# TRI-ML/sdflabel

Hardware: AMD Instinct MI355X
Metric: rendered rays/sec (fwd+bwd) (higher is better)
Workload: dtype f32; 1 GPU; BASELINE configs[1]: one 256x256 crop(s) per GPU, DeepSDF 8x512 on a 40^3 grid, fwd+bwd to yaw/trans/latent, decoder re-evaluated every step; crops_per_gpu=1, rays_per_crop=65536, grid_points=64000, surfels=2751, front_facing=763, parallelism=crop-parallel x1

## Files before the change

### sdflabel_amd/csrc/kcj_slots.h

```cpp
#pragma once
#include <stdint.h>
#if defined(__HIPCC__) || defined(__CUDACC__)
#define SDFR_KCJ_HD __host__ __device__ __forceinline__
#else
#define SDFR_KCJ_HD inline
#endif

constexpr int SDFR_KCJ_PT = 16;
constexpr int SDFR_KCJ_KT = 16;
constexpr int SDFR_KCJ_RING = 4;

SDFR_KCJ_HD int sdfr_kcj_popc(uint32_t x) { return __builtin_popcount(x); }
SDFR_KCJ_HD int sdfr_kcj_count(uint32_t w0, uint32_t w1, uint32_t w2, uint32_t w3) {
    return sdfr_kcj_popc(w0) + sdfr_kcj_popc(w1) + sdfr_kcj_popc(w2) + sdfr_kcj_popc(w3);
}
SDFR_KCJ_HD int sdfr_kcj_rank(uint32_t w0, uint32_t w1, uint32_t w2, uint32_t w3, int q, int g) {
    const uint32_t below = (uint32_t)((1ull << q) - 1ull);
    int r = sdfr_kcj_popc(w0 & below) + sdfr_kcj_popc(w1 & below) + sdfr_kcj_popc(w2 & below) + sdfr_kcj_popc(w3 & below);
    if (g > 0) r += (int)((w0 >> q) & 1u);
    if (g > 1) r += (int)((w1 >> q) & 1u);
    if (g > 2) r += (int)((w2 >> q) & 1u);
    return r;
}
SDFR_KCJ_HD int sdfr_kcj_feature(int q, int g) { return (q >> 2) * 16 + 4 * g + (q & 3); }
SDFR_KCJ_HD int sdfr_kcj_vec(int pos) { return (pos >> 4) * 4 + (pos & 3); }
SDFR_KCJ_HD int sdfr_kcj_comp(int pos) { return (pos & 15) >> 2; }
SDFR_KCJ_HD int sdfr_kcj_elem(int pos, int point) { return (sdfr_kcj_vec(pos) * SDFR_KCJ_PT + point) * 4 + sdfr_kcj_comp(pos); }
SDFR_KCJ_HD int sdfr_kcj_kidx(int pos) { return sdfr_kcj_vec(pos) * 4 + sdfr_kcj_comp(pos); }
SDFR_KCJ_HD int sdfr_kcj_padded(int tot) {
    const int trip = SDFR_KCJ_KT * SDFR_KCJ_RING;
    const int p = (tot + trip - 1) / trip * trip;
    return p < trip ? trip : p;
}
SDFR_KCJ_HD int sdfr_kcj_pad_pos(int tot, int e) { return tot + e / SDFR_KCJ_PT; }
SDFR_KCJ_HD int sdfr_kcj_pad_point(int e) { return e % SDFR_KCJ_PT; }

SDFR_KCJ_HD int sdfr_kcj_col(int j) { return (j & ~127) | ((j & 15) << 3) | ((j >> 4) & 7); }

SDFR_KCJ_HD int sdfr_kcj_ring_clamp(int tile, int nkt) { return tile < nkt ? tile : nkt - 1; }
SDFR_KCJ_HD int sdfr_kcj_ring_gather_tile(int t, int nkt) { return sdfr_kcj_ring_clamp(t + SDFR_KCJ_RING - 1, nkt); }
SDFR_KCJ_HD int sdfr_kcj_ring_klist_tile(int t, int nkt) { return sdfr_kcj_ring_clamp(t + SDFR_KCJ_RING, nkt); }
SDFR_KCJ_HD int sdfr_kcj_ring_operand_tile(int t, int nkt) { return sdfr_kcj_ring_clamp(t + 1, nkt); }
```

### sdflabel_amd/csrc/mlp_kernel.h

```cpp
#pragma once
#include "sdfr_common.h"
#include "kc_slots.h"
#include "kcj_slots.h"
#include "tile_balance.h"
#include <math.h>
#include <type_traits>

typedef float f32x16 __attribute__((ext_vector_type(16)));
typedef float f32x4 __attribute__((ext_vector_type(4)));
typedef _Float16 h16;
typedef h16 h16x8 __attribute__((ext_vector_type(8)));
typedef h16 h16x4 __attribute__((ext_vector_type(4)));

struct MlpLayer {
    int in_dim, out_dim;
    int inj_n, inj_off;
    int kp_f, kp_b, kp_h;
    int off_f, off_b, off_h;
    int kp_bh, off_bh;
    int kp_s, off_s;
    int ln;
};

struct MlpParams {
// ... 106 lines not shown
    static constexpr int KV = 4, NSTEP = 4;
    static __device__ __forceinline__ acc_t step(const vec_t& a, const vec_t& b, acc_t c, int ks) {
        return __builtin_amdgcn_mfma_f32_16x16x4f32(f4c(a, ks), f4c(b, ks), c, 0, 0, 0);
    }
};
template <> struct Mma<h16, 32> {
    typedef f32x16 acc_t; typedef h16x8 vec_t;
    static constexpr int KV = 8, NSTEP = 1;
    static __device__ __forceinline__ acc_t step(const vec_t& a, const vec_t& b, acc_t c, int) {
#ifdef SDFR_ABL_NOMFMA
        c[0] += (float)a[0] * (float)b[0];
        return c;
#else
        return __builtin_amdgcn_mfma_f32_32x32x16_f16(a, b, c, 0, 0, 0);
#endif
    }
};
template <> struct Mma<h16, 16> {
    typedef f32x4 acc_t; typedef h16x8 vec_t;
    static constexpr int KV = 8, NSTEP = 1;
    static __device__ __forceinline__ acc_t step(const vec_t& a, const vec_t& b, acc_t c, int) {
        return __builtin_amdgcn_mfma_f32_16x16x32_f16(a, b, c, 0, 0, 0);
    }
};
__device__ __forceinline__ void store4(float* dst, const float* v) { *reinterpret_cast<float4*>(dst) = make_float4(v[0], v[1], v[2], v[3]); }
__device__ __forceinline__ void store4(h16* dst, const float* v) {
    h16x4 t; t[0] = (h16)v[0]; t[1] = (h16)v[1]; t[2] = (h16)v[2]; t[3] = (h16)v[3];
    *reinterpret_cast<h16x4*>(dst) = t;
}

__device__ __forceinline__ int64_t sdfr_mask_dword(int64_t r, int l, int n_layers, int HP32, int j) {
    return (((r >> 7) * n_layers + l) * 128 + (r & 127)) * HP32 + (j >> 5);
}
__host__ __device__ __forceinline__ int sdfr_wk_row(int r) { return (r & ~63) | ((r & 31) << 1) | ((r >> 5) & 1); }
__device__ __forceinline__ int sdfr_mask_shift(int j) { return ((j >> 2) & 1) * 16 + ((j & 31) >> 3) * 4 + (j & 3); }

#ifndef SDFR_MLP_WPE
#define SDFR_MLP_WPE 1
#endif
template <typename ET, int MS, int FT, int NP, int NW, int MODE, bool LN, int XF> constexpr bool sdfr_mlp_kc() {
    return sizeof(ET) == 4 && MS == 32 && FT == 2 && NP == 2 && NW == 8 && (MODE == 0 || MODE == 1) && !LN && (XF & ~4) == 0;
}
template <typename ET, int MS, int FT, int NP, int NW, int MODE, bool LN, int XF> constexpr bool sdfr_mlp_kcj() {
    return sizeof(ET) == 4 && MS == 16 && NP == 1 && NW == 4 && FT == 8 && MODE == 3 && !LN && XF == 0;
}
template <typename ET, int MS, int FT, int NP, int NW, int PF, int MODE, int PFB_ = 0, bool LN = false, int XF = 0>
__global__ __launch_bounds__(64 * NW, SDFR_MLP_WPE) void sdfr_mlp_kernel(const MlpParams P) {
    typedef Mma<ET, MS> M;
    typedef typename M::acc_t acc_t;
    typedef typename M::vec_t vec_t;
    constexpr bool HALF = sizeof(ET) == 2;
    constexpr bool JAC = MODE == 2 || MODE == 3;
    constexpr bool TAIL = MODE == 4;
    constexpr bool SAVE = MODE == 1;
    constexpr bool LMASK = MODE == 2;
    constexpr bool GMASK = MODE == 3;
    constexpr bool GATHER = (XF & 1) != 0;
    constexpr bool PERSIST = (XF & 2) != 0;
    constexpr bool ORDER = (XF & 4) != 0;
    static_assert(!ORDER || (XF == 4 && (MODE == 0 || MODE == 1) && sizeof(ET) == 4 && MS == 32 && FT == 2), "ORDER: the exact-f32 grid forward alone");
    static_assert(XF == 0 || (MODE == 0 || MODE == 1) || (MODE == 3 && XF == 2), "GATHER is a forward feature; PERSIST: forward modes and the mask-fed Jacobian");
    constexpr bool JPOOL = JAC && PERSIST;
    static_assert(!SAVE || MS == 32, "mask layout assumes 32x32 forward tiles");
    static_assert(!SAVE || (FT * NP) % 2 == 0, "mask words: FT*NP*16 bits per thread and layer must fill whole words");
    static_assert(!HALF || !JAC || MODE == 3, "with half operands only the mask-fed Jacobian exists (MODE 3)");
    static_assert(!LN || (!HALF && MODE != 1 && MODE != 3 && MODE != 4), "LayerNorm decoders: float32 forward (MODE 0) and recomputing Jacobian (MODE 2)");
    static_assert(!TAIL || (NP * MS <= 64 && (NP * MS) % 16 == 0), "tail march: the tile's rows (t_rt rays x K samples) live in wave 0");
    constexpr int KV = M::KV;
    constexpr int NLG = 64 / MS;
    constexpr int RG = MS / (4 * NLG);
    constexpr int KT = KV * NLG;
    constexpr int NT = 64 * NW;
    constexpr int PT = MS * NP;
    constexpr int HP = MS * FT * NW;
    constexpr int KG = HP / KV;
    constexpr int FT32 = HP / (32 * NW);
    constexpr int MW = (FT * NP * RG * 4 + 31) / 32;
    constexpr int MASK_WORDS = LMASK ? (SDFR_MAX_LAYERS * MW * NT) : 1;
    constexpr int LN_F4 = LN ? (NW * PT + SDFR_MAX_LAYERS * PT + 3) / 4 : 0;
    constexpr int KGX = KG + ((HALF && !JAC) ? 4 : 0);
    constexpr bool DBUF = HALF && !JAC && !LN && !SAVE && (2 * KGX * PT * 16 <= 144 * 1024);
    constexpr bool KC = sdfr_mlp_kc<ET, MS, FT, NP, NW, MODE, LN, XF>();
    constexpr int KZ4 = KC ? SDFR_KCD_ROW_BYTES / 16 : 0;
    constexpr int ACT4 = (DBUF ? 2 : 1) * KGX * PT + KZ4;
    constexpr bool MLDS = GMASK && HALF && MS == 16 && HP == 512;
    static_assert(!MLDS || (FT == 4 && NW == 8), "MLDS: a wave owns 64 features = two mask dwords of a row");
    constexpr int MLDS_WORDS = MLDS ? NW * SDFR_MAX_LAYERS * PT * 2 : 0;
    constexpr int O_RED = ACT4, O_ROWS = O_RED + NT / 4, O_GY = O_ROWS + 32, O_SLOTS = O_GY + (PT + 3) / 4, O_MASKS = O_SLOTS + (PT + 3) / 4;
    constexpr int O_LN = O_MASKS + (MASK_WORDS + 3) / 4, O_MLDS = O_LN + LN_F4, LDS4 = O_MLDS + (MLDS_WORDS + 3) / 4;
    __shared__ float4 lds4[LDS4];
    vec_t* act = reinterpret_cast<vec_t*>(lds4);
    ET* act_e = reinterpret_cast<ET*>(lds4);
    vec_t* actw = DBUF ? act + KGX * PT : act;
    ET* actw_e = reinterpret_cast<ET*>(actw);
    float* red = reinterpret_cast<float*>(lds4 + O_RED);
    int* rows = reinterpret_cast<int*>(lds4 + O_ROWS);
    float* gy = reinterpret_cast<float*>(lds4 + O_GY);
    int* slots = reinterpret_cast<int*>(lds4 + O_SLOTS);
    uint32_t* masks = reinterpret_cast<uint32_t*>(lds4 + O_MASKS);
    float* lnred = reinterpret_cast<float*>(lds4 + O_LN);
    float* lnrstd = lnred + NW * PT;
    uint32_t* mlds = reinterpret_cast<uint32_t*>(lds4 + O_MLDS);
    __shared__ float jinj[MLDS ? PT * 8 : 1];
    __shared__ int jpfx[JPOOL ? 66 : 1];
    __shared__ int4 kc_list4[KC ? HP / 4 : 1];
    __shared__ int4 kc_cnt4[KC ? NW / 4 : 1];
    int* kc_cnt = reinterpret_cast<int*>(kc_cnt4);
    static_assert(!KC || (KGX * PT * 16 == SDFR_KCD_ZERO_ROW * SDFR_KCD_ROW_BYTES && HP == SDFR_KCD_WK_ROW_FLOATS),
                  "kc_slots.h: the dense image is 512 rows of 256 bytes, its zero row right behind it");
    static_assert(!KC || (KT == 8 && KV == 4 && NW == 8), "kc_slots.h: k tiles of 8, vectors of 4, 8 waves");
    constexpr bool KCJ = sdfr_mlp_kcj<ET, MS, FT, NP, NW, MODE, LN, XF>();
    __shared__ int4 kcj_list4[KCJ ? HP / 4 : 1];
    __shared__ int4 kcj_cnt4[1];
    static_assert(!KCJ || (KT == SDFR_KCJ_KT && PT == SDFR_KCJ_PT && KV == 4 && PF == SDFR_KCJ_RING && MW == 1), "kcj_slots.h: 16-row tiles, k tiles of 16, ring of 4");

    const int tid = threadIdx.x;
    const int wave = __builtin_amdgcn_readfirstlane(tid >> 6);
    const int lane = tid & 63;
    const int lp = lane % MS;
    const int lg = lane / MS;
    const int NI = P.n_inputs;

#ifdef SDFR_MLP_TRACE
#define SDFR_STAMP(l, i)                                                                                                   \
    do {                                                                                                                   \
        if (P.trace && blockIdx.x == 0 && blockIdx.y == 0 && lane == 0 && wave < 8)                                        \
            P.trace[(wave * SDFR_MAX_LAYERS + (l)) * 5 + (i)] = __builtin_amdgcn_s_memtime();                              \
    } while (0)
#else
#define SDFR_STAMP(l, i) do { } while (0)
#endif
    SDFR_STAMP(8, 0);
#ifdef SDFR_MLP_TRACE
    const bool tt_on = !JAC && !TAIL && P.tile_trace && tid == 0 && blockIdx.y == 0 && (int64_t)blockIdx.x < P.tile_trace_cap;
    if (tt_on) {
        unsigned long long* tt = P.tile_trace + (int64_t)blockIdx.x * SDFR_TILE_TRACE_WORDS;
        tt[0] = __builtin_amdgcn_s_memtime();
        tt[1] = __builtin_amdgcn_s_memrealtime();
        tt[4] = ((unsigned long long)__builtin_amdgcn_s_getreg(20 | (31 << 11)) << 32) | (unsigned long long)__builtin_amdgcn_s_getreg(4 | (31 << 11));
        tt[5] = blockIdx.x;
    }
#endif
    int* tile_slot = reinterpret_cast<int*>(gy) + 1;
    int p_iter = 0, p_live = 0;
    bool p_compact = false;
    if constexpr (PERSIST) {
        if (P.crop_cnt && P.n_crops <= PT) {
            if (tid == 0) {
                int acc_ = 0;
                for (int c = 0; c < P.n_crops; ++c) {
                    const int64_t cc = min((int64_t)P.crop_cnt[c], P.crop_rows);
                    acc_ += (int)((cc + PT - 1) / PT);
                    slots[c] = acc_;
                }
                tile_slot[1] = acc_;
            }
            __syncthreads();
            p_live = tile_slot[1];
            p_compact = true;
            if ((int)blockIdx.x >= p_live) return;
        } else if (P.skip && !P.crop_cnt) {
            bool any = false;
            for (int c = 0; c < P.n_crops; ++c) any = any || P.skip[c] == 0;
            if (!any) return;
        }
        if constexpr (JPOOL) {
            if (tid == 0) {
                int acc_ = 0;
                for (int c = 0; c < P.n_crops; ++c) { acc_ += (sdfr_count(P.cnt, c, P.cap) + PT - 1) / PT; jpfx[c] = acc_; }
                jpfx[64] = acc_;
            }
            __syncthreads();
            p_live = jpfx[64];
            if ((int)blockIdx.x >= p_live) return;
        }
    }
    do {
    int tile = blockIdx.x;
    if constexpr (PERSIST) {
        const int64_t j = (int64_t)blockIdx.x + (int64_t)p_iter * gridDim.x;
        ++p_iter;
        if constexpr (JPOOL) {
            if (j >= p_live) return;
            tile = (int)j;
        } else
        if (p_compact) {
            if (j >= p_live) return;
            int lo = 0, hi = P.n_crops - 1;
            while (lo < hi) { const int mid = (lo + hi) >> 1; if (slots[mid] > (int)j) hi = mid; else lo = mid + 1; }
            const int before = lo > 0 ? slots[lo - 1] : 0;
            tile = (int)((int64_t)lo * (P.crop_rows / PT) + (j - before));
        } else {
            if (j * PT >= P.n) return;
            tile = (int)j;
        }
        if (p_iter > 1) __syncthreads();
    }
// ... 398 lines not shown
                kk &= 8 * SDFR_KCD_ROW_BYTES - 1;
#endif
                const float2 w = *reinterpret_cast<const float2*>(reinterpret_cast<const char*>(Wl) + (uint32_t)(sdfr_kcd_weight_byte(kk) + wlane4));
                const float2 v = *reinterpret_cast<const float2*>(reinterpret_cast<const char*>(act_e) + sdfr_kcd_operand_byte(kk, lp));
                aa[0][ks] = w.x;
                aa[FT - 1][ks] = w.y;
                bb[0][ks] = v.x;
                bb[NP - 1][ks] = v.y;
            };
            auto mma1 = [&](const vec_t* aa, const vec_t* bb, int ks) {
#pragma unroll
                for (int f = 0; f < FT; ++f)
#pragma unroll
                    for (int p = 0; p < NP; ++p) acc[f][p] = M::step(aa[f], bb[p], acc[f][p], ks);
            };
            ko[0] = klp[0];
            ko[1] = klp[sdfr_kc_ring_clamp(1, nkt) * NLG];
#pragma unroll
            for (int ks = 0; ks < M::NSTEP; ++ks) { load_a1(ko[0], ks, a[0], b[0]); __builtin_amdgcn_sched_barrier(0); }
#pragma unroll
            for (int ks = 0; ks < M::NSTEP; ++ks) { load_a1(ko[1], ks, a[1], b[1]); __builtin_amdgcn_sched_barrier(0); }
            ko[0] = klp[sdfr_kc_ring_clamp(2, nkt) * NLG];
            ko[1] = klp[sdfr_kc_ring_clamp(3, nkt) * NLG];
#pragma unroll
            for (int f = 0; f < FT; ++f)
#pragma unroll
                for (int p = 0; p < NP; ++p)
#pragma unroll
                    for (int r = 0; r < RG * 4; ++r) acc[f][p][r] = 0.f;
            __builtin_amdgcn_sched_barrier(0);
            for (int t = 0; t < nkt; t += SDFR_KC_RING_STAGES) {
#pragma unroll
                for (int u = 0; u < SDFR_KC_RING_STAGES; ++u) {
                    const int s = sdfr_kc_ring_stage(u);
#pragma unroll
                    for (int ks = 0; ks < M::NSTEP; ++ks) {
                        mma1(a[s], b[s], ks);
                        __builtin_amdgcn_sched_barrier(0);
                        load_a1(ko[s], ks, a[s], b[s]);
                        __builtin_amdgcn_sched_barrier(0);
                    }
                    ko[s] = klp[sdfr_kc_ring_klist_tile(t + u, nkt) * NLG];
                }
            }
            return;
        }
        const int last = nkt - 1;
        ko[0] = klp[0];
        load_a(ko[0], a[0]);
        load_b(ko[0], b[0]);
        ko[1] = klp[min(1, last) * NLG];
        for (int t = 0; t < nkt; t += 2) {
            load_a(ko[1], a[1]);
            load_b(ko[1], b[1]);
            ko[0] = klp[min(t + 2, last) * NLG];
            __builtin_amdgcn_sched_barrier(0);
            mma(a[0], b[0]);
            __builtin_amdgcn_sched_barrier(0);
            load_a(ko[0], a[0]);
            load_b(ko[0], b[0]);
            ko[1] = klp[min(t + 3, last) * NLG];
            __builtin_amdgcn_sched_barrier(0);
            mma(a[1], b[1]);
            __builtin_amdgcn_sched_barrier(0);
        }
    };
    auto gemm_kc = [&](auto Wl, int nk, int rows_active) {
        int nact = (rows_active - fbase + MS - 1) / MS;
        nact = nact < 0 ? 0 : (nact > FT ? FT : nact);
        nact = __builtin_amdgcn_readfirstlane(nact);
        if (nact != FT || nk < KT) {
#pragma unroll
            for (int f = 0; f < FT; ++f)
#pragma unroll
                for (int p = 0; p < NP; ++p)
#pragma unroll
                    for (int r = 0; r < RG * 4; ++r) acc[f][p][r] = 0.f;
        }
        if (nact == FT) gemm_kc_body(Wl, nk, FT, std::true_type{});
        else if (nact > 0) gemm_kc_body(Wl, nk, nact, std::false_type{});
    };
    auto gemm_kcj = [&](const float* __restrict__ Wl, int nk) {
        if constexpr (KCJ) {
        const int nkt = nk / KT;
        const uint32_t wlane4 = (uint32_t)(fbase + 8 * lp) * 4u;
        const vec_t* bptr = act + lg * PT + lp;
        const int4* klp = kcj_list4 + lg;
        float4 a[SDFR_KCJ_RING][4][2], b[2];
        auto load_a = [&](const int4& k, float4 (*aa)[2]) {
#pragma unroll
            for (int ks = 0; ks < 4; ++ks) {
                const int kk = ks == 0 ? k.x : ks == 1 ? k.y : ks == 2 ? k.z : k.w;
                const float4* wp = reinterpret_cast<const float4*>(reinterpret_cast<const char*>(Wl) + (uint32_t)((uint32_t)kk * 4u + wlane4));
                aa[ks][0] = wp[0];
                aa[ks][1] = wp[1];
            }
        };
        int4 ko = klp[0];
#pragma unroll
        for (int u = 0; u < SDFR_KCJ_RING - 1; ++u) {
            load_a(ko, a[u]);
            ko = klp[sdfr_kcj_ring_clamp(u + 1, nkt) * NLG];
        }
        b[0] = bptr[0];
#pragma unroll
        for (int f = 0; f < FT; ++f)
#pragma unroll
            for (int r = 0; r < 4; ++r) acc[f][0][r] = 0.f;
        __builtin_amdgcn_sched_barrier(0);
        for (int t = 0; t < nkt; t += SDFR_KCJ_RING) {
#pragma unroll
            for (int u = 0; u < SDFR_KCJ_RING; ++u) {
                load_a(ko, a[(u + SDFR_KCJ_RING - 1) % SDFR_KCJ_RING]);
                b[(u + 1) % 2] = bptr[sdfr_kcj_ring_operand_tile(t + u, nkt) * (NLG * PT)];
                ko = klp[sdfr_kcj_ring_klist_tile(t + u, nkt) * NLG];
                __builtin_amdgcn_sched_barrier(0);
#pragma unroll
                for (int ks = 0; ks < 4; ++ks)
#pragma unroll
                    for (int f = 0; f < FT; ++f)
                        acc[f][0] = __builtin_amdgcn_mfma_f32_16x16x4f32(f4c(a[u][ks][f >> 2], f & 3), f4c(b[u % 2], ks), acc[f][0], 0, 0, 0);
                __builtin_amdgcn_sched_barrier(0);
            }
        }
        }
    };
    auto feat0 = [&](int f, int rg) { return fbase + f * MS + rg * (4 * NLG) + 4 * lg; };
    const vec_t* Wfwd = reinterpret_cast<const vec_t*>(HALF ? (const void*)P.Wh : (const void*)P.Wf);

    auto point_sums = [&](float* v) {
#pragma unroll
        for (int p = 0; p < NP; ++p) {
            float x = v[p];
            for (int o = MS; o < 64; o <<= 1) x += __shfl_xor(x, o, 64);
            if (lg == 0) lnred[wave * PT + p * MS + lp] = x;
        }
        __syncthreads();
#pragma unroll
        for (int p = 0; p < NP; ++p) {
            float t = 0.f;
#pragma unroll
            for (int w = 0; w < NW; ++w) t += lnred[w * PT + p * MS + lp];
            v[p] = t;
        }
        __syncthreads();
    };
    const int64_t wg_lin = (int64_t)blockIdx.y * gridDim.x + blockIdx.x;
    auto ln_forward = [&](int l, int n_out) {
        const float* bias = P.bias + l * HP;
        const float* gam = P.ln_gamma + l * HP;
        const float* bet = P.ln_beta + l * HP;
        float s1[NP], mu[NP], rs[NP];
#pragma unroll
        for (int p = 0; p < NP; ++p) s1[p] = 0.f;
#pragma unroll
        for (int f = 0; f < FT; ++f)
#pragma unroll
            for (int r = 0; r < RG * 4; ++r) {
                const int j = feat0(f, r >> 2) + (r & 3);
#pragma unroll
                for (int p = 0; p < NP; ++p) {
                    const float x = (j < n_out) ? acc[f][p][r] + bias[j] : 0.f;
                    acc[f][p][r] = x;
                    s1[p] += x;
                }
            }
        point_sums(s1);
#pragma unroll
        for (int p = 0; p < NP; ++p) { mu[p] = s1[p] / (float)n_out; s1[p] = 0.f; }
#pragma unroll
        for (int f = 0; f < FT; ++f)
#pragma unroll
            for (int r = 0; r < RG * 4; ++r) {
                const int j = feat0(f, r >> 2) + (r & 3);
#pragma unroll
                for (int p = 0; p < NP; ++p)
                    if (j < n_out) { const float d = acc[f][p][r] - mu[p]; s1[p] += d * d; }
            }
        point_sums(s1);
#pragma unroll
        for (int p = 0; p < NP; ++p) rs[p] = 1.f / sqrtf(s1[p] / (float)n_out + 1e-5f);
#pragma unroll
        for (int f = 0; f < FT; ++f)
#pragma unroll
            for (int rg = 0; rg < RG; ++rg) {
                const int j0 = feat0(f, rg);
#pragma unroll
                for (int p = 0; p < NP; ++p) {
                    float xh[4];
#pragma unroll
                    for (int i = 0; i < 4; ++i) {
                        const int j = j0 + i;
                        xh[i] = (j < n_out) ? (acc[f][p][rg * 4 + i] - mu[p]) * rs[p] : 0.f;
                        acc[f][p][rg * 4 + i] = (j < n_out) ? xh[i] * gam[j] + bet[j] : 0.f;
                    }
                    if (JAC) P.ln_ws[((wg_lin * P.n_mfma + l) * (HP / 4) + (j0 >> 2)) * PT + p * MS + lp] = make_float4(xh[0], xh[1], xh[2], xh[3]);
                }
            }
        if (JAC && lg == 0 && wave == 0) {
#pragma unroll
            for (int p = 0; p < NP; ++p) lnrstd[l * PT + p * MS + lp] = rs[p];
        }
    };

    int* t_more = reinterpret_cast<int*>(gy);
    const bool kc_on = KC && P.kcompact && P.Wk;
// ... 328 lines not shown
                    atomicAdd(P.tile_cost + sdfr_tb_cost_index(P.tile_at[place], place, P.gather_rows), rows[127]);
                }
            } else {
                if (tid < n_valid) {
                    const int64_t row = (int64_t)tile * PT + tid;
                    if (!P.skip || !P.skip[row / P.skip_rows]) P.sdf[row] = o;
                }
            }
        }
    }
#ifdef SDFR_MLP_TRACE
    if (tt_on) {
        unsigned long long* tt = P.tile_trace + (int64_t)blockIdx.x * SDFR_TILE_TRACE_WORDS;
        tt[2] = __builtin_amdgcn_s_memtime();
        tt[3] = __builtin_amdgcn_s_memrealtime();
    }
#endif
    if constexpr (TAIL) {
        --t_left;
        if (tid == 0) *t_more = 0;
        __syncthreads();
        if (t_act && t_left > 0) *t_more = 1;
        __syncthreads();
        if (*t_more == 0) break;
        ++t_pass;
        tail_rows(pass_k(P.t_step0 + t_pass), false);
        __syncthreads();
        build_operand();
        __syncthreads();
    }
    } while (TAIL);
    if constexpr (TAIL) {
        if (tid < 64) {
            const unsigned long long left_over = __ballot(t_act && tid < RT);
            const bool hand_over = P.t_next_cnt && (P.t_stage < P.t_steps);
            int base = 0;
            if (tid == 0) {
                if (P.t_evals) atomicAdd(P.t_evals, t_ev);
                if (left_over && !hand_over && P.t_unresolved) atomicAdd(P.t_unresolved, (int)__popcll(left_over));
                if (left_over && hand_over) base = atomicAdd(P.t_next_cnt, (int)__popcll(left_over));
            }
            if (hand_over && left_over) {
                base = __shfl(base, 0, 64);
                if (t_act && tid < RT) {
                    const int at = base + (int)__popcll(left_over & ((1ull << tid) - 1ull));
                    P.t_next_pix[at] = t_gp;
                    P.t_next_lam[at] = t_st;
                }
            }
        }
        if (!P.t_tile_ctr) return;
        continue;
    }
    if constexpr (JAC) {
    uint32_t raw[NP * FT * RG];
    const bool kcj_on = KCJ && P.jcompact && P.Wkj;
    uint32_t kcj_w[4] = {0u, 0u, 0u, 0u};
    int kcj_n = 0;
    auto kcj_vote = [&](int l, const uint32_t* raw) {
        const int prev_out = P.L[l - 1].out_dim;
        uint32_t m = 0u;
#pragma unroll
        for (int f = 0; f < FT; ++f) m |= ((raw[f] >> sdfr_mask_shift(fbase + f * MS + 4 * lg)) & 0xFu) << (4 * f);
        if (__builtin_amdgcn_readfirstlane((int)(fbase + MS * FT > prev_out)) != 0) {
            uint32_t keep = 0u;
#pragma unroll
            for (int f = 0; f < FT; ++f) {
                const int nv = min(max(prev_out - (fbase + f * MS + 4 * lg), 0), 4);
                keep |= ((1u << nv) - 1u) << (4 * f);
            }
            m &= keep;
        }
        int x = (int)m;
        x |= __builtin_amdgcn_update_dpp(0, x, 0xB1, 0xf, 0xf, false);
        x |= __builtin_amdgcn_update_dpp(0, x, 0x4E, 0xf, 0xf, false);
        x |= __builtin_amdgcn_update_dpp(0, x, 0x124, 0xf, 0xf, false);
        x |= __builtin_amdgcn_update_dpp(0, x, 0x128, 0xf, 0xf, false);
#pragma unroll
        for (int g = 0; g < 4; ++g) kcj_w[g] = (uint32_t)__builtin_amdgcn_readlane(x, 16 * g);
        if (lane == 0) reinterpret_cast<int*>(kcj_cnt4)[wave] = sdfr_kcj_count(kcj_w[0], kcj_w[1], kcj_w[2], kcj_w[3]);
    };
    const bool kcj_top = kcj_on && P.n_mfma >= 2;
    if constexpr (KCJ) {
        if (kcj_top) {
            const int r = rows[lp];
#pragma unroll
            for (int f = 0; f < FT; ++f) raw[f] = P.maskbuf[sdfr_mask_dword(r, P.n_mfma - 1, P.n_mfma, HP / 32, fbase + f * MS + 4 * lg)];
            kcj_vote(P.n_mfma, raw);
        }
    }
    __syncthreads();
    SDFR_STAMP(8, 2);

    auto mask_addr = [&](int j, int r, int l, int& shift) -> int64_t {
        shift = sdfr_mask_shift(j);
        return sdfr_mask_dword(r, l - 1, P.n_mfma, HP / 32, j);
    };
    auto fetch_masks = [&](int l, uint32_t* raw) {
#pragma unroll
        for (int p = 0; p < NP; ++p) {
            const int r = rows[p * MS + lp];
#pragma unroll
            for (int f = 0; f < FT; ++f)
#pragma unroll
                for (int rg = 0; rg < RG; ++rg) {
                    int shift;
                    raw[(p * FT + f) * RG + rg] = P.maskbuf[mask_addr(feat0(f, rg), r, l, shift)];
                }
        }
    };
    auto store_in_grad = [&](int l, const uint32_t* raw, auto&& value) {
        const MlpLayer L = P.L[l];
        const int prev_out = P.L[l - 1].out_dim;
        const int inj_hi = prev_out + L.inj_n;
        if constexpr (MLDS) {
            const uint2* mst = reinterpret_cast<const uint2*>(mlds) + ((int64_t)wave * SDFR_MAX_LAYERS + (l - 1)) * PT;
            const int msh = (lg & 1) * 16 + (lg >> 1) * 4;
            uint32_t mk[NP][2];
#pragma unroll
            for (int p = 0; p < NP; ++p) {
                const uint2 m2 = mst[p * MS + lp];
                mk[p][0] = m2.x >> msh; mk[p][1] = m2.y >> msh;
            }
#pragma unroll
            for (int f = 0; f < FT; ++f) {
                const int j0 = feat0(f, 0);
                const bool tail_f = __builtin_amdgcn_readfirstlane((int)(fbase + (f + 1) * MS > prev_out)) != 0;
#pragma unroll
                for (int p = 0; p < NP; ++p) {
                    const int pt = p * MS + lp;
                    float v[4];
#pragma unroll
                    for (int i = 0; i < 4; ++i) {
                        const float x = value(f, p, 0, i, j0 + i, pt);
                        const int m = __builtin_amdgcn_sbfe((int)mk[p][f >> 1], (f & 1) * 8 + i, 1);
                        v[i] = __int_as_float(__float_as_int(x) & m);
                    }
                    if (tail_f) {
#pragma unroll
                        for (int i = 0; i < 4; ++i) {
                            const int k = j0 + i;
                            if (k >= prev_out) {
                                if (k < inj_hi) {
                                    if (jdir) jinj[pt * 8 + L.inj_off + (k - prev_out)] += value(f, p, 0, i, k, pt);
                                    else if (slots[pt] >= 0) atomicAdd(P.J + (int64_t)slots[pt] * NI + L.inj_off + (k - prev_out), value(f, p, 0, i, k, pt));
                                }
                                v[i] = 0.f;
                            }
                        }
                    }
                    store4(act_e + ((j0 / KV) * PT + pt) * KV + (j0 % KV), v);
                }
            }
            return;
        }
        uint32_t mw[MW];
        if (GMASK) {
#pragma unroll
            for (int w = 0; w < MW; ++w) mw[w] = 0u;
#pragma unroll
            for (int p = 0; p < NP; ++p) {
                const int r = rows[p * MS + lp];
#pragma unroll
                for (int f = 0; f < FT; ++f)
#pragma unroll
                    for (int rg = 0; rg < RG; ++rg) {
// ... 15 lines not shown
            for (int f = 0; f < FT; ++f)
#pragma unroll
                for (int rg = 0; rg < RG; ++rg) {
                    const int j0 = feat0(f, rg);
#pragma unroll
                    for (int p = 0; p < NP; ++p) {
                        const int pt = p * MS + lp;
#pragma unroll
                        for (int i = 0; i < 4; ++i) {
                            const int k = j0 + i;
                            const int bit = ((f * NP + p) * RG + rg) * 4 + i;
                            float x = value(f, p, rg, i, k, pt);
                            if (!TAIL || k < prev_out) {
                                x = ((mw[bit >> 5] >> (bit & 31)) & 1u) ? x : 0.f;
                            } else {
                                if (k < inj_hi && slots[pt] >= 0)
                                    atomicAdd(P.J + (int64_t)slots[pt] * NI + L.inj_off + (k - prev_out), x);
                                x = 0.f;
                            }
                            acc[f][p][rg * 4 + i] = x;
                        }
                    }
                }
        };
        if (tail_here) apply_masks(std::true_type{});
        else apply_masks(std::false_type{});
        if constexpr (LN) {
            if (P.L[l - 1].ln) {
                const float* gam = P.ln_gamma + (l - 1) * HP;
                const float4* xh4 = P.ln_ws + ((wg_lin * P.n_mfma + (l - 1)) * (HP / 4)) * PT;
                float s1[NP], s2[NP];
#pragma unroll
                for (int p = 0; p < NP; ++p) { s1[p] = 0.f; s2[p] = 0.f; }
#pragma unroll
                for (int f = 0; f < FT; ++f)
#pragma unroll
                    for (int rg = 0; rg < RG; ++rg) {
                        const int j0 = feat0(f, rg);
#pragma unroll
                        for (int p = 0; p < NP; ++p) {
                            const float4 xh = xh4[(j0 >> 2) * PT + p * MS + lp];
#pragma unroll
                            for (int i = 0; i < 4; ++i) {
                                const int k = j0 + i;
                                const float gh = (k < prev_out) ? acc[f][p][rg * 4 + i] * gam[k] : 0.f;
                                acc[f][p][rg * 4 + i] = gh;
                                s1[p] += gh;
                                s2[p] += gh * f4c(xh, i);
                            }
                        }
                    }
                point_sums(s1);
                point_sums(s2);
#pragma unroll
                for (int f = 0; f < FT; ++f)
#pragma unroll
                    for (int rg = 0; rg < RG; ++rg) {
                        const int j0 = feat0(f, rg);
#pragma unroll
                        for (int p = 0; p < NP; ++p) {
                            const float4 xh = xh4[(j0 >> 2) * PT + p * MS + lp];
                            const float rs = lnrstd[(l - 1) * PT + p * MS + lp];
                            const float m1 = s1[p] / (float)prev_out, m2 = s2[p] / (float)prev_out;
#pragma unroll
                            for (int i = 0; i < 4; ++i)
                                acc[f][p][rg * 4 + i] = (j0 + i < prev_out) ? rs * (acc[f][p][rg * 4 + i] - m1 - f4c(xh, i) * m2) : 0.f;
                        }
                    }
            }
        }
        if constexpr (KCJ) {
            if (kcj_on && l >= 2) {
                const int4 c4 = kcj_cnt4[0];
                const int c[4] = {c4.x, c4.y, c4.z, c4.w};
                int off = 0, tot = 0;
#pragma unroll
                for (int w = 0; w < 4; ++w) {
                    off += w < wave ? c[w] : 0;
                    tot += c[w];
                }
                off = __builtin_amdgcn_readfirstlane(off);
                tot = __builtin_amdgcn_readfirstlane(tot);
                const uint32_t mine = lg == 0 ? kcj_w[0] : lg == 1 ? kcj_w[1] : lg == 2 ? kcj_w[2] : kcj_w[3];
                int n = off;
#pragma unroll
                for (int q = 0; q < 32; ++q) {
                    const int b0 = (int)((kcj_w[0] >> q) & 1u), b1 = (int)((kcj_w[1] >> q) & 1u), b2 = (int)((kcj_w[2] >> q) & 1u),
                              b3 = (int)((kcj_w[3] >> q) & 1u);
                    const int front = ((b0 << 2) | ((b0 + b1) << 4) | ((b0 + b1 + b2) << 6)) >> (2 * lg) & 3;
                    if ((mine >> q) & 1u) act_e[sdfr_kcj_elem(n + front, lp)] = acc[q >> 2][0][q & 3];
                    n += b0 + b1 + b2 + b3;
                }
#pragma unroll
                for (int h = 0; h < 2; ++h) {
                    const int q = lp + 16 * h;
                    if ((mine >> q) & 1u)
                        reinterpret_cast<int*>(kcj_list4)[sdfr_kcj_kidx(off + sdfr_kcj_rank(kcj_w[0], kcj_w[1], kcj_w[2], kcj_w[3], q, lg))] =
                            (fbase + sdfr_kcj_feature(q, lg)) * HP;
                }
                const int padded = sdfr_kcj_padded(tot);
                for (int e = tid; e < (padded - tot) * PT; e += NT) {
                    const int pos = sdfr_kcj_pad_pos(tot, e);
                    act_e[sdfr_kcj_elem(pos, sdfr_kcj_pad_point(e))] = 0.f;
                    if (sdfr_kcj_pad_point(e) == 0) reinterpret_cast<int*>(kcj_list4)[sdfr_kcj_kidx(pos)] = 0;
                }
                kcj_n = padded;
                return;
            }
        }
#pragma unroll
        for (int f = 0; f < FT; ++f)
#pragma unroll
            for (int rg = 0; rg < RG; ++rg) {
                const int j0 = feat0(f, rg);
#pragma unroll
                for (int p = 0; p < NP; ++p) {
                    float v[4];
#pragma unroll
                    for (int i = 0; i < 4; ++i) v[i] = acc[f][p][rg * 4 + i];
                    store4(act_e + ((j0 / KV) * PT + p * MS + lp) * KV + (j0 % KV), v);
                }
            }
    };

    if (GMASK && !MLDS && !kcj_top) fetch_masks(P.n_mfma, raw);
    SDFR_STAMP(8, 3);
    if constexpr (MLDS) {
        if (P.n_mfma >= 1 && !(P.n_mfma - 1 == 0 && P.L[0].in_dim <= 8))
            preload_a(reinterpret_cast<const vec_t*>(P.Wbh) + P.L[P.n_mfma - 1].off_bh);
        float4 wl[FT];
        float gyp[NP];
#pragma unroll
        for (int f = 0; f < FT; ++f) wl[f] = *reinterpret_cast<const float4*>(P.w_last + feat0(f, 0));
#pragma unroll
        for (int p = 0; p < NP; ++p) gyp[p] = gy[p * MS + lp];
        store_in_grad(P.n_mfma, raw, [&](int f, int p, int, int i, int, int) { return f4c(wl[f], i) * gyp[p]; });
    } else
    store_in_grad(P.n_mfma, raw, [&](int, int, int, int, int k, int pt) { return P.w_last[k] * gy[pt]; });
    __syncthreads();
    SDFR_STAMP(8, 4);
    for (int l = P.n_mfma - 1; l >= 0; --l) {
        const MlpLayer L = P.L[l];
        if constexpr (MLDS) {
          if (l == 0 && L.in_dim <= 8) {
            constexpr int TPW = (HP / KT) / NW;
            const vec_t* Wl = reinterpret_cast<const vec_t*>(P.Wbh) + L.off_bh;
            const int nkt = L.kp_bh / KT;
            acc_t a0[NP];
            vec_t av[TPW], bv[TPW][NP];
            SDFR_STAMP(9, 0);
#pragma unroll
            for (int u = 0; u < TPW; ++u) {
                const int t = wave * TPW + u;
#pragma unroll
                for (int i = 0; i < KV; ++i) av[u][i] = (ET)0;
                if (t < nkt) av[u] = Wl[(int64_t)(t * NLG + lg) * HP + lp];
#pragma unroll
                for (int p = 0; p < NP; ++p) bv[u][p] = act[(t * NLG + lg) * PT + p * MS + lp];
            }
#pragma unroll
            for (int p = 0; p < NP; ++p) {
#pragma unroll
                for (int r = 0; r < 4; ++r) a0[p][r] = 0.f;
#pragma unroll
                for (int u = 0; u < TPW; ++u) a0[p] = M::step(av[u], bv[u][p], a0[p], 0);
            }
            SDFR_STAMP(9, 1);
            float* part = reinterpret_cast<float*>(mlds);
            if (lg < 2) {
#pragma unroll
                for (int p = 0; p < NP; ++p)
                    *reinterpret_cast<float4*>(part + ((wave * PT + p * MS + lp) * 8 + 4 * lg)) = make_float4(a0[p][0], a0[p][1], a0[p][2], a0[p][3]);
            }
            __syncthreads();
            for (int e = tid; e < 8 * PT; e += NT) {
                const int q = e >> 3, k = e & 7;
                float t = 0.f;
#pragma unroll
                for (int w = 0; w < NW; ++w) t += part[(w * PT + q) * 8 + k];
                if (k < NI && slots[q] >= 0) {
                    if (k >= L.in_dim) t = 0.f;
                    if (jdir) P.J[(int64_t)slots[q] * NI + k] = jinj[q * 8 + k] + t;
                    else atomicAdd(P.J + (int64_t)slots[q] * NI + k, t);
                }
            }
            SDFR_STAMP(9, 2);
            break;
          }
        }
        if (!MLDS && l == 0 && L.in_dim <= 8) {
// ... 127 lines not shown
```

Baseline: 56.39 million rays/s.

## Gather sparse MLP operands from the dense activation tile instead of compacting them

The compacted-Jacobian GEMM now keeps activations in the normal dense LDS layout. Each k-list entry holds a raw feature index, and the GEMM reads both the weight row and the matching activation scalar through that index. The per-layer scatter of surviving activations into a packed buffer goes away. Padding entries point at a zero group placed right after the operand tile, and padding shrinks from four k-tiles to two. A head-peeled 4-stage ring handles tile counts that are not a multiple of four. In exchange, the B operand is now fetched as four scalar LDS loads per tile instead of one vector load, which may add LDS traffic and latency on the MFMA chain.

```diff
diff --git a/sdflabel_amd/csrc/kcj_slots.h b/sdflabel_amd/csrc/kcj_slots.h
--- a/sdflabel_amd/csrc/kcj_slots.h
+++ b/sdflabel_amd/csrc/kcj_slots.h
@@ -41,3 +41,27 @@
 SDFR_KCJ_HD int sdfr_kcj_ring_gather_tile(int t, int nkt) { return sdfr_kcj_ring_clamp(t + SDFR_KCJ_RING - 1, nkt); }
 SDFR_KCJ_HD int sdfr_kcj_ring_klist_tile(int t, int nkt) { return sdfr_kcj_ring_clamp(t + SDFR_KCJ_RING, nkt); }
 SDFR_KCJ_HD int sdfr_kcj_ring_operand_tile(int t, int nkt) { return sdfr_kcj_ring_clamp(t + 1, nkt); }
+
+constexpr int SDFR_KCJD_HP = 512;
+constexpr int SDFR_KCJD_ZERO = SDFR_KCJD_HP;
+constexpr int SDFR_KCJD_ZERO_VECS = SDFR_KCJ_PT;
+constexpr int SDFR_KCJD_TRIP_TILES = 2;
+SDFR_KCJ_HD int sdfr_kcjd_entry(int feature) { return feature; }
+SDFR_KCJ_HD int sdfr_kcjd_pad_entry() { return SDFR_KCJD_ZERO; }
+SDFR_KCJ_HD int sdfr_kcjd_padded(int tot) {
+    const int trip = SDFR_KCJ_KT * SDFR_KCJD_TRIP_TILES;
+    const int p = (tot + trip - 1) / trip * trip;
+    return p < trip ? trip : p;
+}
+SDFR_KCJ_HD int sdfr_kcjd_pad_pos(int tot, int i) { return tot + i; }
+SDFR_KCJ_HD uint32_t sdfr_kcjd_operand_byte(int e, int lp) { return (uint32_t)((((e >> 2) * SDFR_KCJ_PT + lp) * 4 + (e & 3)) * 4); }
+SDFR_KCJ_HD uint32_t sdfr_kcjd_weight_byte(int e) { return (uint32_t)(e & (SDFR_KCJD_HP - 1)) * (uint32_t)(SDFR_KCJD_HP * 4); }
+constexpr int SDFR_KCJD_OPERAND_BYTES = (SDFR_KCJD_HP / 4 + 1) * SDFR_KCJ_PT * 16;
+constexpr int SDFR_KCJD_IMAGE_BYTES = SDFR_KCJD_HP * SDFR_KCJD_HP * 4;
+constexpr int SDFR_KCJD_STAGES = 4, SDFR_KCJD_LEAD = 3, SDFR_KCJD_HEAD = 2;
+SDFR_KCJ_HD int sdfr_kcjd_ring_clamp(int tile, int nkt) { return tile < nkt ? tile : nkt - 1; }
+SDFR_KCJ_HD bool sdfr_kcjd_ring_head(int nkt) { return (nkt & SDFR_KCJD_HEAD) != 0; }
+SDFR_KCJ_HD int sdfr_kcjd_ring_stage(int tile, int nkt) { return (tile + (nkt & SDFR_KCJD_HEAD)) % SDFR_KCJD_STAGES; }
+SDFR_KCJ_HD int sdfr_kcjd_ring_gather_tile(int t, int nkt) { return sdfr_kcjd_ring_clamp(t + SDFR_KCJD_LEAD, nkt); }
+SDFR_KCJ_HD int sdfr_kcjd_ring_klist_tile(int t, int nkt) { return sdfr_kcjd_ring_clamp(t + SDFR_KCJD_LEAD + 1, nkt); }
+SDFR_KCJ_HD int sdfr_kcjd_ring_operand_tile(int t, int nkt) { return sdfr_kcjd_ring_gather_tile(t, nkt); }
diff --git a/sdflabel_amd/csrc/mlp_kernel.h b/sdflabel_amd/csrc/mlp_kernel.h
--- a/sdflabel_amd/csrc/mlp_kernel.h
+++ b/sdflabel_amd/csrc/mlp_kernel.h
@@ -212,7 +212,8 @@
     constexpr bool DBUF = HALF && !JAC && !LN && !SAVE && (2 * KGX * PT * 16 <= 144 * 1024);
     constexpr bool KC = sdfr_mlp_kc<ET, MS, FT, NP, NW, MODE, LN, XF>();
     constexpr int KZ4 = KC ? SDFR_KCD_ROW_BYTES / 16 : 0;
-    constexpr int ACT4 = (DBUF ? 2 : 1) * KGX * PT + KZ4;
+    constexpr int KJZ4 = sdfr_mlp_kcj<ET, MS, FT, NP, NW, MODE, LN, XF>() ? SDFR_KCJD_ZERO_VECS : 0;
+    constexpr int ACT4 = (DBUF ? 2 : 1) * KGX * PT + KZ4 + KJZ4;
     constexpr bool MLDS = GMASK && HALF && MS == 16 && HP == 512;
     static_assert(!MLDS || (FT == 4 && NW == 8), "MLDS: a wave owns 64 features = two mask dwords of a row");
     constexpr int MLDS_WORDS = MLDS ? NW * SDFR_MAX_LAYERS * PT * 2 : 0;
@@ -243,6 +244,7 @@
     __shared__ int4 kcj_list4[KCJ ? HP / 4 : 1];
     __shared__ int4 kcj_cnt4[1];
     static_assert(!KCJ || (KT == SDFR_KCJ_KT && PT == SDFR_KCJ_PT && KV == 4 && PF == SDFR_KCJ_RING && MW == 1), "kcj_slots.h: 16-row tiles, k tiles of 16, ring of 4");
+    static_assert(!KCJ || (HP == SDFR_KCJD_HP && ACT4 * 16 == SDFR_KCJD_OPERAND_BYTES), "kcj_slots.h: the zero group lies right behind the 512-feature operand tile");
 
     const int tid = threadIdx.x;
     const int wave = __builtin_amdgcn_readfirstlane(tid >> 6);
@@ -807,46 +809,63 @@
     };
     auto gemm_kcj = [&](const float* __restrict__ Wl, int nk) {
         if constexpr (KCJ) {
+        constexpr int R = SDFR_KCJD_STAGES;
         const int nkt = nk / KT;
         const uint32_t wlane4 = (uint32_t)(fbase + 8 * lp) * 4u;
-        const vec_t* bptr = act + lg * PT + lp;
         const int4* klp = kcj_list4 + lg;
-        float4 a[SDFR_KCJ_RING][4][2], b[2];
-        auto load_a = [&](const int4& k, float4 (*aa)[2]) {
+        float4 a[R][4][2];
+        float b[R][4];
+        auto load_ab = [&](const int4& k, float4 (*aa)[2], float* bb) {
 #pragma unroll
             for (int ks = 0; ks < 4; ++ks) {
-                const int kk = ks == 0 ? k.x : ks == 1 ? k.y : ks == 2 ? k.z : k.w;
-                const float4* wp = reinterpret_cast<const float4*>(reinterpret_cast<const char*>(Wl) + (uint32_t)((uint32_t)kk * 4u + wlane4));
+                const int e = ks == 0 ? k.x : ks == 1 ? k.y : ks == 2 ? k.z : k.w;
+                const float4* wp = reinterpret_cast<const float4*>(reinterpret_cast<const char*>(Wl) + (uint32_t)(sdfr_kcjd_weight_byte(e) + wlane4));
                 aa[ks][0] = wp[0];
                 aa[ks][1] = wp[1];
+                bb[ks] = *reinterpret_cast<const float*>(reinterpret_cast<const char*>(act_e) + sdfr_kcjd_operand_byte(e, lp));
             }
         };
         int4 ko = klp[0];
-#pragma unroll
-        for (int u = 0; u < SDFR_KCJ_RING - 1; ++u) {
-            load_a(ko, a[u]);
-            ko = klp[sdfr_kcj_ring_clamp(u + 1, nkt) * NLG];
-        }
-        b[0] = bptr[0];
-#pragma unroll
-        for (int f = 0; f < FT; ++f)
-#pragma unroll
-            for (int r = 0; r < 4; ++r) acc[f][0][r] = 0.f;
-        __builtin_amdgcn_sched_barrier(0);
-        for (int t = 0; t < nkt; t += SDFR_KCJ_RING) {
-#pragma unroll
-            for (int u = 0; u < SDFR_KCJ_RING; ++u) {
-                load_a(ko, a[(u + SDFR_KCJ_RING - 1) % SDFR_KCJ_RING]);
-                b[(u + 1) % 2] = bptr[sdfr_kcj_ring_operand_tile(t + u, nkt) * (NLG * PT)];
-                ko = klp[sdfr_kcj_ring_klist_tile(t + u, nkt) * NLG];
-                __builtin_amdgcn_sched_barrier(0);
-#pragma unroll
-                for (int ks = 0; ks < 4; ++ks)
-#pragma unroll
-                    for (int f = 0; f < FT; ++f)
-                        acc[f][0] = __builtin_amdgcn_mfma_f32_16x16x4f32(f4c(a[u][ks][f >> 2], f & 3), f4c(b[u % 2], ks), acc[f][0], 0, 0, 0);
-                __builtin_amdgcn_sched_barrier(0);
-            }
+        auto chain_tile = [&](int tile, int u) {
+            load_ab(ko, a[(u + R - 1) % R], b[(u + R - 1) % R]);
+            ko = klp[sdfr_kcjd_ring_klist_tile(tile, nkt) * NLG];
+            __builtin_amdgcn_sched_barrier(0);
+#pragma unroll
+            for (int ks = 0; ks < 4; ++ks)
+#pragma unroll
+                for (int f = 0; f < FT; ++f)
+                    acc[f][0] = __builtin_amdgcn_mfma_f32_16x16x4f32(f4c(a[u][ks][f >> 2], f & 3), b[u][ks], acc[f][0], 0, 0, 0);
+            __builtin_amdgcn_sched_barrier(0);
+        };
+        auto zero_acc = [&]() {
+#pragma unroll
+            for (int f = 0; f < FT; ++f)
+#pragma unroll
+                for (int r = 0; r < 4; ++r) acc[f][0][r] = 0.f;
+            __builtin_amdgcn_sched_barrier(0);
+        };
+        int t = 0;
+        if (sdfr_kcjd_ring_head(nkt)) {
+#pragma unroll
+            for (int u = 0; u < R - 1; ++u) {
+                load_ab(ko, a[(u + SDFR_KCJD_HEAD) % R], b[(u + SDFR_KCJD_HEAD) % R]);
+                ko = klp[sdfr_kcjd_ring_clamp(u + 1, nkt) * NLG];
+            }
+            zero_acc();
+#pragma unroll
+            for (int u = 0; u < SDFR_KCJD_HEAD; ++u) chain_tile(u, (u + SDFR_KCJD_HEAD) % R);
+            t = SDFR_KCJD_HEAD;
+        } else {
+#pragma unroll
+            for (int u = 0; u < R - 1; ++u) {
+                load_ab(ko, a[u], b[u]);
+                ko = klp[sdfr_kcjd_ring_clamp(u + 1, nkt) * NLG];
+            }
+            zero_acc();
+        }
+        for (; t < nkt; t += R) {
+#pragma unroll
+            for (int u = 0; u < R; ++u) chain_tile(t + u, u);
         }
         }
     };
@@ -1341,6 +1360,7 @@
     };
     const bool kcj_top = kcj_on && P.n_mfma >= 2;
     if constexpr (KCJ) {
+        if (kcj_on && tid < KJZ4) lds4[KGX * PT + tid] = make_float4(0.f, 0.f, 0.f, 0.f);
         if (kcj_top) {
             const int r = rows[lp];
 #pragma unroll
@@ -1522,30 +1542,16 @@
                 off = __builtin_amdgcn_readfirstlane(off);
                 tot = __builtin_amdgcn_readfirstlane(tot);
                 const uint32_t mine = lg == 0 ? kcj_w[0] : lg == 1 ? kcj_w[1] : lg == 2 ? kcj_w[2] : kcj_w[3];
-                int n = off;
-#pragma unroll
-                for (int q = 0; q < 32; ++q) {
-                    const int b0 = (int)((kcj_w[0] >> q) & 1u), b1 = (int)((kcj_w[1] >> q) & 1u), b2 = (int)((kcj_w[2] >> q) & 1u),
-                              b3 = (int)((kcj_w[3] >> q) & 1u);
-                    const int front = ((b0 << 2) | ((b0 + b1) << 4) | ((b0 + b1 + b2) << 6)) >> (2 * lg) & 3;
-                    if ((mine >> q) & 1u) act_e[sdfr_kcj_elem(n + front, lp)] = acc[q >> 2][0][q & 3];
-                    n += b0 + b1 + b2 + b3;
-                }
 #pragma unroll
                 for (int h = 0; h < 2; ++h) {
                     const int q = lp + 16 * h;
                     if ((mine >> q) & 1u)
                         reinterpret_cast<int*>(kcj_list4)[sdfr_kcj_kidx(off + sdfr_kcj_rank(kcj_w[0], kcj_w[1], kcj_w[2], kcj_w[3], q, lg))] =
-                            (fbase + sdfr_kcj_feature(q, lg)) * HP;
-                }
-                const int padded = sdfr_kcj_padded(tot);
-                for (int e = tid; e < (padded - tot) * PT; e += NT) {
-                    const int pos = sdfr_kcj_pad_pos(tot, e);
-                    act_e[sdfr_kcj_elem(pos, sdfr_kcj_pad_point(e))] = 0.f;
-                    if (sdfr_kcj_pad_point(e) == 0) reinterpret_cast<int*>(kcj_list4)[sdfr_kcj_kidx(pos)] = 0;
-                }
+                            sdfr_kcjd_entry(fbase + sdfr_kcj_feature(q, lg));
+                }
+                const int padded = sdfr_kcjd_padded(tot);
+                if (tid < padded - tot) reinterpret_cast<int*>(kcj_list4)[sdfr_kcj_kidx(sdfr_kcjd_pad_pos(tot, tid))] = sdfr_kcjd_pad_entry();
                 kcj_n = padded;
-                return;
             }
         }
 #pragma unroll
```

Result: no change. 56.86 million rays/s (median of 6 runs) (+0.8%).
